# DIAGNijmegen/prostateMR_3D-CAD-csPCa

Hardware: AMD Instinct MI355X
Metric: train-step volumes/sec (whole job), M1 (20,160,160,3) (higher is better)
Workload: dtype bf16; 1 GPU; C3 M1 full hierarchical-probabilistic dense_skip+deep_supervision latents (3,2,1,0) (20,160,160,3); batch_per_gpu=2, global_batch=2, params=67254246, parallelism=dp1, hip_graph=True

## Files before the change

### prostatemr_3d-cad-cspca_amd/csrc/wgrad_tf.hip

```cpp
#include "common.h"
#include "gather.h"
#include <stdlib.h>

typedef __attribute__((ext_vector_type(8))) __bf16 bf16x8_t;
typedef __attribute__((ext_vector_type(4))) float f32x4_t;
typedef short s16x4_t __attribute__((ext_vector_type(4)));
typedef const __attribute__((address_space(1))) void* gptr_t;
typedef __attribute__((address_space(3))) void* lptr_t;

__device__ __attribute__((aligned(64))) unsigned int m1_zero_page_w[16];

__device__ __forceinline__ void glds16w(const void* g, void* lds_wave_base) {
    __builtin_amdgcn_global_load_lds((gptr_t)g, (lptr_t)lds_wave_base, 16, 0, 0);
}
__device__ __forceinline__ s16x4_t tr_read(const unsigned char* p) {
    return __builtin_amdgcn_ds_read_tr16_b64_v4i16((__attribute__((address_space(3))) s16x4_t*)p);
}

#define TF_MAX_NKS 4
#define TF_MAX_AIT 10

struct TfP {
    const bf16_t* A; const bf16_t* B; float* R; float* bsum;
    int CA, CB, AD, AH, AW, BD, BH, BW, N;
    long long RT, RSA; int a_off, b_off;
    int sd, sh, sw, pd, ph, pw;
    int KWs, TH;
    int AHt, AWt;
    int spra, sprb;
    int a_slots, b_slots;
    int a_bytes, b_bytes;
    int tiles_w, tiles_h; long long ntiles;
    int bTiles, nsplit;
    int stages;
    float* Rx; long long rx_stride;
    long long rx_bias;
    int nks;
    int nmem; const bf16_t* Am[M1_MAX_SRC]; long long rx_mem;
};

typedef unsigned u32x2_t __attribute__((ext_vector_type(2)));
__device__ __forceinline__ u32x2_t tr_read_asm(unsigned lds_addr) {
    u32x2_t v;
    asm volatile("ds_read_b64_tr_b16 %0, %1" : "=v"(v) : "v"(lds_addr) : "memory");
    return v;
}
__device__ __forceinline__ void lds_wait2(u32x2_t& a, u32x2_t& b) { asm volatile("s_waitcnt lgkmcnt(0)" : "+v"(a), "+v"(b)); }
__device__ __forceinline__ bf16x8_t frag8(u32x2_t lo, u32x2_t hi) {
    return __builtin_bit_cast(bf16x8_t, __builtin_shufflevector(lo, hi, 0, 1, 2, 3));
}
__device__ __forceinline__ void wait_vm(int n) {
    switch (n) {
#define TF_W(N_) case N_: asm volatile("s_waitcnt vmcnt(" #N_ ")" ::: "memory"); break;
        TF_W(0) TF_W(1) TF_W(2) TF_W(3) TF_W(4) TF_W(5) TF_W(6) TF_W(7) TF_W(8) TF_W(9) TF_W(10) TF_W(11) TF_W(12)
        TF_W(13) TF_W(14) TF_W(15) TF_W(16) TF_W(17) TF_W(18) TF_W(19) TF_W(20) TF_W(21) TF_W(22) TF_W(23) TF_W(24)
        TF_W(25) TF_W(26) TF_W(27) TF_W(28) TF_W(29) TF_W(30) TF_W(31) TF_W(32) TF_W(33) TF_W(34) TF_W(35) TF_W(36)
        TF_W(37) TF_W(38) TF_W(39) TF_W(40) TF_W(41) TF_W(42) TF_W(43) TF_W(44) TF_W(45) TF_W(46) TF_W(47) TF_W(48)
#undef TF_W
        default: asm volatile("s_waitcnt vmcnt(0)" ::: "memory"); break;
    }
}

#define TF_MAX_STAGES 8

template <int KD, int KH, int KW, int KPARTS, int TF_NKS>
__global__ void __launch_bounds__(256) wgrad_tf_kernel(TfP p) {
#if defined(__HIP_DEVICE_COMPILE__)
    constexpr int NT = KD * KH * KW, NG = KD * KH;
    extern __shared__ __attribute__((aligned(16))) unsigned char smem[];
    const int tid = threadIdx.x, lane = tid & 63, wave = __builtin_amdgcn_readfirstlane(tid >> 6);
    constexpr int kparts = KPARTS, ntile = 4 / KPARTS;
    const int ntb = p.CB > 16 ? 2 : 1;
    const int tile_id = wave % ntile, part = wave / ntile;
    const int ta = tile_id / ntb, tb = tile_id % ntb;
    const int a0 = (blockIdx.x / p.bTiles) * 32, b0 = (blockIdx.x % p.bTiles) * 32;
    const int mem = p.nmem > 1 ? (int)blockIdx.z : 0;
    const bf16_t* Abase = p.A;
    if (p.nmem > 1) {
        Abase = p.Am[0];
#pragma unroll
        for (int m = 1; m < M1_MAX_SRC; ++m) if (mem == m) Abase = p.Am[m];
    }
    const int PA = p.spra * 16, PB = p.sprb * 16;
    const int stage_bytes = p.a_bytes + p.b_bytes;
    const unsigned char* zero_pg = reinterpret_cast<const unsigned char*>(m1_zero_page_w);

    constexpr unsigned OOB = 0x80000000u;
    unsigned a_vo[TF_MAX_AIT]; int a_pk[TF_MAX_AIT];
    const int nait = p.a_slots >> 8;
#pragma unroll
    for (int it = 0; it < TF_MAX_AIT; ++it) {
        const int q = it * 256 + tid;
        const int row = q / p.spra, slp = q - row * p.spra;
        const int dd = row / (p.AHt * p.AWt); const int r2 = row - dd * (p.AHt * p.AWt);
        const int hh = r2 / p.AWt, ww = r2 - hh * p.AWt;
        const int sl = p.spra == 4 ? (slp ^ (((ww >> 3) & 1) << 1)) : slp;
        a_pk[it] = dd | (hh << 8) | (ww << 16);
        a_vo[it] = (row < KD * p.AHt * p.AWt) ? (unsigned)((((dd * p.AH + hh) * p.AW + ww) * p.CA + a0 + sl * 8) * 2) : OOB;
    }
    constexpr int NBIT = (TF_NKS * 32 * 4 + 255) / 256;
    const int nbit = (p.b_slots + 255) >> 8;
    unsigned b_vo[NBIT]; int b_th[NBIT];
#pragma unroll
    for (int it = 0; it < NBIT; ++it) {
        const int q = it * 256 + tid;
        const int row = q / p.sprb, slp = q - row * p.sprb;
        const int th = row / p.KWs, tw = row - th * p.KWs;
        const int sl = p.sprb == 4 ? (slp ^ (((tw >> 3) & 1) << 1)) : slp;
        b_th[it] = th;
        b_vo[it] = q < p.b_slots ? (unsigned)(((th * p.BW + tw) * p.CB + b0 + sl * 8) * 2) : OOB;
    }

    int q_kt = blockIdx.y, q_tw, q_th, q_bd, q_n;
    { int r = q_kt; q_tw = r % p.tiles_w; r /= p.tiles_w; q_th = r % p.tiles_h; r /= p.tiles_h; q_bd = r % p.BD; q_n = r / p.BD; }
    int s_tw, s_th, s_bd, s_n;
    { int r = p.nsplit; s_tw = r % p.tiles_w; r /= p.tiles_w; s_th = r % p.tiles_h; r /= p.tiles_h; s_bd = r % p.BD; s_n = r / p.BD; }
    auto issue = [&](int st) {
        const bool live = q_kt < (int)p.ntiles;
        const int twi = q_tw, thi = q_th, bd = q_bd, n = q_n;
        q_kt += p.nsplit;
        q_tw += s_tw; int c = q_tw >= p.tiles_w; q_tw -= c ? p.tiles_w : 0;
        q_th += s_th + c; c = q_th >= p.tiles_h; q_th -= c ? p.tiles_h : 0;
        q_bd += s_bd + c; c = q_bd >= p.BD; q_bd -= c ? p.BD : 0;
        q_n += s_n + c;
        const int ad0 = bd * p.sd - p.pd, ah0 = thi * p.TH * p.sh - p.ph, aw0 = twi * p.KWs * p.sw - p.pw;
        const long long lin0 = (((long long)n * p.AD + ad0) * p.AH + ah0) * p.AW + aw0;
        const int bh0 = thi * p.TH;
        const long long blin0 = (((long long)n * p.BD + bd) * p.BH + bh0) * p.BW + twi * p.KWs;
        unsigned char* As = smem + st * stage_bytes;
        unsigned char* Bs = As + p.a_bytes;
        const __amdgpu_buffer_rsrc_t ra = __builtin_amdgcn_make_buffer_rsrc((void*)(Abase + lin0 * p.CA), 0, live ? 0x7fffffff : 0, 0x00020000);
        const __amdgpu_buffer_rsrc_t rb = __builtin_amdgcn_make_buffer_rsrc((void*)(p.B + blin0 * p.CB), 0, live ? 0x7fffffff : 0, 0x00020000);
        const bool a_inner = ad0 >= 0 && ad0 + KD - 1 < p.AD && ah0 >= 0 && ah0 + p.AHt - 1 < p.AH && aw0 >= 0 && aw0 + p.AWt - 1 < p.AW;
        if (a_inner) {
#pragma unroll
            for (int it = 0; it < TF_MAX_AIT; ++it)
                if (it < nait) __builtin_amdgcn_raw_ptr_buffer_load_lds(ra, (lptr_t)(As + (it * 256 + wave * 64) * 16), 16, a_vo[it], 0, 0, 0);
        } else {
#pragma unroll
            for (int it = 0; it < TF_MAX_AIT; ++it) {
                if (it < nait) {
                    const int pk = a_pk[it];
                    const int dd = pk & 0xff, hh = (pk >> 8) & 0xff, ww = (pk >> 16) & 0xff;
                    const bool ok = (unsigned)(ad0 + dd) < (unsigned)p.AD && (unsigned)(ah0 + hh) < (unsigned)p.AH && (unsigned)(aw0 + ww) < (unsigned)p.AW;
                    __builtin_amdgcn_raw_ptr_buffer_load_lds(ra, (lptr_t)(As + (it * 256 + wave * 64) * 16), 16, ok ? a_vo[it] : OOB, 0, 0, 0);
                }
            }
        }
        const bool b_inner = bh0 + p.TH <= p.BH;
#pragma unroll
        for (int it = 0; it < NBIT; ++it)
            if (it < nbit)
                __builtin_amdgcn_raw_ptr_buffer_load_lds(rb, (lptr_t)(Bs + (it * 256 + wave * 64) * 16), 16,
                                                         (b_inner || bh0 + b_th[it] < p.BH) ? b_vo[it] : OOB, 0, 0, 0);
    };

    const int g = lane >> 4, i = lane & 15;
    const unsigned lds0 = (unsigned)(unsigned long long)(lptr_t)smem;
    unsigned a_ad[TF_NKS][2][KW], b_ad[TF_NKS][2];
#pragma unroll
    for (int ks = 0; ks < TF_NKS; ++ks)
#pragma unroll
        for (int h = 0; h < 2; ++h) {
            const int kk = ks * 32 + 8 * g + 4 * h + (i >> 2);
            const int th = kk / p.KWs, tw = kk - th * p.KWs;
#pragma unroll
            for (int kw = 0; kw < KW; ++kw) {
                const int ww = tw * p.sw + kw;
                const int half = p.spra == 4 ? (ta ^ ((ww >> 3) & 1)) : ta;
                a_ad[ks][h][kw] = lds0 + ((th * p.sh) * p.AWt + ww) * PA + half * 32 + (i & 3) * 8;
            }
            const int halfb = p.sprb == 4 ? (tb ^ ((tw >> 3) & 1)) : tb;
            b_ad[ks][h] = lds0 + p.a_bytes + kk * PB + halfb * 32 + (i & 3) * 8;
        }
    const int grp_pitch = p.AWt * PA;

    f32x4_t acc[NT];
#pragma unroll
    for (int t = 0; t < NT; ++t) acc[t] = (f32x4_t){0.f, 0.f, 0.f, 0.f};
    const bool do_bsum = p.bsum != nullptr && a0 == 0 && ta == 0 && part == 0 && mem == 0;
    f32x4_t accb = (f32x4_t){0.f, 0.f, 0.f, 0.f};
    const bf16x8_t ones = __builtin_bit_cast(bf16x8_t, make_uint4(0x3F803F80u, 0x3F803F80u, 0x3F803F80u, 0x3F803F80u));

    const int S = p.stages;
    const int npiece = nait + nbit;
    const long long kt0 = blockIdx.y, step = p.nsplit;
    for (int s = 0; s < S - 1; ++s) issue(s);
    int st = 0;
    for (long long kt = kt0; kt < p.ntiles; kt += step) {
        wait_vm(npiece * (S - 2));
        __builtin_amdgcn_s_barrier();
        int stn = st + S - 1; if (stn >= S) stn -= S;
        issue(stn);
        const unsigned sb = (unsigned)(st * stage_bytes);
        constexpr int NU = TF_NKS * KD, CH = KH * KW;
        u32x2_t bl[2], bh[2], al[2][CH], ah[2][CH];
        auto rd_unit = [&](int u, int set) {
            const int ks = u / KD, kd = u % KD;
            if (kd == 0) { bl[ks & 1] = tr_read_asm(b_ad[ks][0] + sb); bh[ks & 1] = tr_read_asm(b_ad[ks][1] + sb); }
#pragma unroll
            for (int kh = 0; kh < KH; ++kh) {
                const unsigned ro = sb + (unsigned)((kd * p.AHt + kh) * grp_pitch);
#pragma unroll
                for (int kw = 0; kw < KW; ++kw) {
                    if (((kd * CH + kh * KW + kw) % kparts) == part) {
                        al[set][kh * KW + kw] = tr_read_asm(a_ad[ks][0][kw] + ro);
                        ah[set][kh * KW + kw] = tr_read_asm(a_ad[ks][1][kw] + ro);
                    }
                }
            }
        };
        rd_unit(0, 0);
#pragma unroll
        for (int u = 0; u < NU; ++u) {
            const int ks = u / KD, kd = u % KD, set = u & 1;
            if (kd == 0) lds_wait2(bl[ks & 1], bh[ks & 1]);
#pragma unroll
            for (int c = 0; c < CH; ++c) lds_wait2(al[set][c], ah[set][c]);
            if (u + 1 < NU) rd_unit(u + 1, set ^ 1);
            __builtin_amdgcn_sched_barrier(0);
            const bf16x8_t bfr = frag8(bl[ks & 1], bh[ks & 1]);
            if (do_bsum && kd == 0) accb = __builtin_amdgcn_mfma_f32_16x16x32_bf16(ones, bfr, accb, 0, 0, 0);
#pragma unroll
            for (int c = 0; c < CH; ++c)
                if (((kd * CH + c) % kparts) == part)
                    acc[kd * CH + c] = __builtin_amdgcn_mfma_f32_16x16x32_bf16(frag8(al[set][c], ah[set][c]), bfr, acc[kd * CH + c], 0, 0, 0);
            __builtin_amdgcn_sched_barrier(0);
        }
        if (++st == S) st = 0;
    }
    asm volatile("s_waitcnt vmcnt(0)" ::: "memory");

    float* Rx = p.Rx + (long long)mem * p.rx_mem + (long long)blockIdx.y * p.rx_stride;
    const int b = b0 + tb * 16 + i;
    if (do_bsum && g == 0 && b < p.CB) Rx[p.rx_bias + b] = accb[0];
#pragma unroll
    for (int t = 0; t < NT; ++t)
#pragma unroll
        for (int r = 0; r < 4; ++r) {
            const int a = a0 + ta * 16 + g * 4 + r;
            if ((t % kparts) == part && a < p.CA && b < p.CB) Rx[((long long)t * p.CA + a) * p.CB + b] = acc[t][r];
        }
#endif
}


struct TfFin { float* Rx; long long stride; int ncopies; float* R; int NT, CA, CB; long long RT, RSA; int a_off, b_off;
               float* bsum; long long rx_bias; int nb; int EL; int bias_serial; };
__device__ __forceinline__ void tf_fold_generic(const TfFin& f, unsigned vb, float* red) {
    const long long n = (long long)f.NT * f.CA * f.CB;
    const int e = threadIdx.x % f.EL, y = threadIdx.x / f.EL, YL = 256 / f.EL;
    const long long i = (long long)vb * f.EL + e;
    const long long idx = i;
    float* dst = nullptr;
    if (i < n) {
        const int b = (int)(i % f.CB); const long long q = i / f.CB; const int a = (int)(q % f.CA), t = (int)(q / f.CA);
        dst = f.R + (long long)t * f.RT + (long long)(a + f.a_off) * f.RSA + b + f.b_off;
    } else if (i < n + f.nb) { dst = f.bsum + (i - n) + f.b_off; }
    float s = 0.f;
    if (dst) {
#pragma unroll 8
        for (int c = y; c < f.ncopies; c += YL) s += f.Rx[(long long)c * f.stride + idx];
    }
    red[threadIdx.x] = s;
    __syncthreads();
    if (y == 0 && dst) {
        for (int q = 1; q < YL; ++q) s += red[q * f.EL + e];
        *dst += s;
    }
}
__global__ void __launch_bounds__(256) tf_finish_kernel(TfFin f) {
    __shared__ float red[256];
    tf_fold_generic(f, blockIdx.x, red);
}

__device__ __forceinline__ void tf_fold_vec(const TfFin& f, unsigned vb, unsigned nblk) {
    const long long n = (long long)f.NT * f.CA * f.CB, n4 = n >> 2;
    for (long long q = (long long)vb * 256 + threadIdx.x; q < n4; q += (long long)nblk * 256) {
        const long long i = q << 2;
        float4 s = *reinterpret_cast<const float4*>(f.Rx + i);
        for (int c = 1; c < f.ncopies; ++c) {
            const float4 v = *reinterpret_cast<const float4*>(f.Rx + (long long)c * f.stride + i);
            s.x += v.x; s.y += v.y; s.z += v.z; s.w += v.w;
        }
        const int b = (int)(i % f.CB); const long long r = i / f.CB; const int a = (int)(r % f.CA), t = (int)(r / f.CA);
        float* dst = f.R + (long long)t * f.RT + (long long)(a + f.a_off) * f.RSA + b + f.b_off;
        dst[0] += s.x; dst[1] += s.y; dst[2] += s.z; dst[3] += s.w;
    }
    if (vb == 0)
        for (int j = threadIdx.x; j < f.nb; j += 256) {
            float s = 0.f;
            for (int c = 0; c < f.ncopies; ++c) s += f.Rx[(long long)c * f.stride + n + j];
            f.bsum[j + f.b_off] += s;
        }
}
__global__ void __launch_bounds__(256) tf_finish_vec_kernel(TfFin f) { tf_fold_vec(f, blockIdx.x, gridDim.x); }

__device__ __forceinline__ void tf_fold_wide(const TfFin& f, unsigned vb, float4 (*red)[64]) {
    const long long n = (long long)f.NT * f.CA * f.CB;
    const int lane = threadIdx.x & 63, w = threadIdx.x >> 6;
    const long long i = ((long long)vb * 64 + lane) << 2;
    float4 s = make_float4(0.f, 0.f, 0.f, 0.f);
    if (i < n) {
#pragma unroll 4
        for (int c = w; c < f.ncopies; c += 4) {
            const float4 v = *reinterpret_cast<const float4*>(f.Rx + (long long)c * f.stride + i);
            s.x += v.x; s.y += v.y; s.z += v.z; s.w += v.w;
        }
    }
    red[w][lane] = s;
    __syncthreads();
    if (w == 0 && i < n) {
#pragma unroll
        for (int q = 1; q < 4; ++q) { const float4 v = red[q][lane]; s.x += v.x; s.y += v.y; s.z += v.z; s.w += v.w; }
        const int b = (int)(i % f.CB); const long long r = i / f.CB; const int a = (int)(r % f.CA), t = (int)(r / f.CA);
        float* dst = f.R + (long long)t * f.RT + (long long)(a + f.a_off) * f.RSA + b + f.b_off;
        dst[0] += s.x; dst[1] += s.y; dst[2] += s.z; dst[3] += s.w;
    }
    if (vb == 0 && f.bias_serial) {
        for (int j = threadIdx.x; j < f.nb; j += 256) {
            float sb = 0.f;
            for (int c = 0; c < f.ncopies; ++c) sb += f.Rx[(long long)c * f.stride + n + j];
            f.bsum[j + f.b_off] += sb;
        }
    } else if (vb == 0 && f.nb > 0) {
        __syncthreads();
        float* const rb = reinterpret_cast<float*>(red);
        int nbp = 1; while (nbp < f.nb && nbp < 256) nbp <<= 1;
        const int rows = 256 / nbp, j = threadIdx.x % nbp, r0 = threadIdx.x / nbp;
        for (int j0 = 0; j0 < f.nb; j0 += nbp) {
            float sb = 0.f;
            if (j0 + j < f.nb) {
#pragma unroll 4
                for (int c = r0; c < f.ncopies; c += rows) sb += f.Rx[(long long)c * f.stride + n + j0 + j];
            }
            rb[threadIdx.x] = sb;
            __syncthreads();
            if (r0 == 0 && j0 + j < f.nb) {
                for (int q = 1; q < rows; ++q) sb += rb[q * nbp + j];
                f.bsum[j0 + j + f.b_off] += sb;
            }
            __syncthreads();
        }
    }
}
__global__ void __launch_bounds__(256) tf_finish_wide_kernel(TfFin f) {
    __shared__ float4 red[4][64];
    tf_fold_wide(f, blockIdx.x, red);
}

#define TF_FOLD_MAX 24
struct TfFoldBatch { int n; int pref[TF_FOLD_MAX + 1]; int mode[TF_FOLD_MAX]; TfFin f[TF_FOLD_MAX]; };
static_assert(sizeof(TfFoldBatch) <= 3800, "fold batch must fit the kernel argument segment");
__global__ void __launch_bounds__(256) tf_finish_batch_kernel(TfFoldBatch B) {
    __shared__ float4 red[4][64];
    int j = 0;
    while (j + 1 < B.n && (int)blockIdx.x >= B.pref[j + 1]) ++j;
    const unsigned vb = blockIdx.x - B.pref[j], nblk = B.pref[j + 1] - B.pref[j];
    const TfFin& f = B.f[j];
    if (B.mode[j] == 1) tf_fold_vec(f, vb, nblk);
    else if (B.mode[j] == 2) tf_fold_wide(f, vb, red);
    else tf_fold_generic(f, vb, reinterpret_cast<float*>(red));
}

static inline bool tf_chan_ok(int c) { return c == 8 || c == 16 || (c >= 32 && c % 32 == 0); }

static bool tf_plan(const WgradSpec& g, TfP& p) {
    if (g.dtype != M1_BF16) return false;
    const bool k133 = g.kd == 1 && g.kh == 3 && g.kw == 3, k333 = g.kd == 3 && g.kh == 3 && g.kw == 3;
    if (!k133 && !k333) return false;
    if (!tf_chan_ok(g.CA) || !tf_chan_ok(g.CB)) return false;
    if (g.BW % 8) return false;
    if ((long long)g.N * g.AD * g.AH * g.AW >= (1ll << 31) - (1 << 20) || (long long)g.N * g.BD * g.BH * g.BW >= (1ll << 31) - (1 << 20)) return false;
    p = TfP{};
    p.A = (const bf16_t*)g.A; p.B = (const bf16_t*)g.B; p.R = g.R; p.bsum = g.bsum;
    p.CA = g.CA; p.CB = g.CB; p.AD = g.AD; p.AH = g.AH; p.AW = g.AW; p.BD = g.BD; p.BH = g.BH; p.BW = g.BW; p.N = g.N;
    p.RT = g.RT; p.RSA = g.RSA; p.a_off = g.a_off; p.b_off = g.b_off;
    p.sd = g.sd; p.sh = g.sh; p.sw = g.sw; p.pd = g.pd; p.ph = g.ph; p.pw = g.pw;
    p.KWs = g.BW % 32 == 0 ? 32 : (g.BW % 16 == 0 ? 16 : 8);
    int n4 = M1_CFG("M1_TF_NKS4", 2);
    const int nks = ((n4 && g.CA <= 16 && g.CB <= 16) || (n4 == 2 && g.kd == 1)) ? 4 : 2;
    p.nks = nks;
    p.TH = nks * (32 / p.KWs);
    p.AHt = (p.TH - 1) * g.sh + g.kh; p.AWt = (p.KWs - 1) * g.sw + g.kw;
    p.spra = (g.CA < 32 ? g.CA : 32) / 8; p.sprb = (g.CB < 32 ? g.CB : 32) / 8;
    const int a_rows = g.kd * p.AHt * p.AWt;
    p.a_slots = (a_rows * p.spra + 255) / 256 * 256; p.b_slots = nks * 32 * p.sprb;
    if (p.a_slots > TF_MAX_AIT * 256 || p.AHt > 255 || p.AWt > 255) return false;
    p.a_bytes = p.a_slots * 16; p.b_bytes = (p.b_slots + 255) / 256 * 256 * 16 + 64;
    p.tiles_w = g.BW / p.KWs; p.tiles_h = (g.BH + p.TH - 1) / p.TH;
    p.ntiles = (long long)g.N * g.BD * p.tiles_h * p.tiles_w;
    if (p.ntiles >= (1ll << 30)) return false;
    const int sb = p.a_bytes + p.b_bytes, npiece = p.a_slots / 256 + (p.b_slots + 255) / 256;
    int S = (76 * 1024) / sb;
    if (S < 3) S = 3;
    if (S > TF_MAX_STAGES) S = TF_MAX_STAGES;
    while (S > 3 && npiece * (S - 2) > 48) --S;
    { int fs = M1_CFG("M1_TF_STAGES", 0); if (fs >= 3) S = fs; }
    p.stages = S;
    return npiece * (S - 2) <= 48 && (size_t)S * sb <= 160 * 1024;
}
bool m1_tf_wgrad_supported(const WgradSpec& g) { TfP p; return tf_plan(g, p); }

#include <mutex>
#include <vector>
struct TfPending { TfFin f; int mode; int blocks; };
static std::mutex g_fold_mu;
static std::vector<TfPending> g_fold_pending;
static int g_fold_defer = 0;
static int fold_launch_pending_locked(hipStream_t st) {
    size_t i = 0;
    while (i < g_fold_pending.size()) {
        TfFoldBatch B{}; B.pref[0] = 0;
        while (i < g_fold_pending.size() && B.n < TF_FOLD_MAX) {
            const TfPending& q = g_fold_pending[i++];
            B.f[B.n] = q.f; B.mode[B.n] = q.mode; B.pref[B.n + 1] = B.pref[B.n] + q.blocks; ++B.n;
        }
        hipLaunchKernelGGL(tf_finish_batch_kernel, dim3((unsigned)B.pref[B.n]), dim3(256), 0, st, B);
        int rc = m1_check_launch(); if (rc) { g_fold_pending.clear(); return rc; }
    }
    g_fold_pending.clear();
    return M1_OK;
}
int m1_fold_defer_set(int on) { std::lock_guard<std::mutex> lk(g_fold_mu); const int was = g_fold_defer; g_fold_defer = on ? 1 : 0; return was; }
extern "C" int m1_wgrad_defer(int on) { std::lock_guard<std::mutex> lk(g_fold_mu); g_fold_defer = on ? 1 : 0; return M1_OK; }
int m1_fold_defer_get() { std::lock_guard<std::mutex> lk(g_fold_mu); return g_fold_defer; }
extern "C" int m1_wgrad_fold_drop(void) { { std::lock_guard<std::mutex> lk(g_fold_mu); g_fold_pending.clear(); } m1_colsum_drop_pending(); return M1_OK; }
extern "C" int m1_wgrad_fold_pending(void* stream) {
    if (m1_debug_skip("fold")) return m1_wgrad_fold_drop();
    {
        std::lock_guard<std::mutex> lk(g_fold_mu);
        const int rc = fold_launch_pending_locked((hipStream_t)stream); if (rc) return rc;
    }
    return m1_colsum_launch_pending((hipStream_t)stream);
}

int m1_wg_rx_finish(float* rx, long long stride, int ncopies, const WgradSpec& g, long long nw, hipStream_t st) {
    TfFin f{rx, stride, ncopies, g.R, g.kd * g.kh * g.kw, g.CA, g.CB, g.RT, g.RSA, g.a_off, g.b_off, g.bsum, nw, g.bsum ? g.CB : 0, 32,
            M1_CFG("M1_TF_BIAS_SERIAL", 0)};
    const long long n = (long long)f.NT * f.CA * f.CB + f.nb;
    int mode = 0; long long blocks;
    if (ncopies <= 16 && f.CB % 4 == 0 && n >= (1 << 16)) {
        mode = 1; blocks = (n / 4 + 255) / 256; if (blocks > 4096) blocks = 4096;
    } else if (f.CB % 4 == 0 && n - f.nb >= (1 << 15)) {
        mode = 2; blocks = (n - f.nb + 255) / 256;
    } else {
        while (f.EL > 4 && n / f.EL < 128) f.EL >>= 1;
        blocks = (n + f.EL - 1) / f.EL;
    }
    {
        std::lock_guard<std::mutex> lk(g_fold_mu);
        if (g_fold_defer) {
            bool dup = false;
            for (const TfPending& q : g_fold_pending)
                if (q.f.R == f.R && q.f.a_off == f.a_off && q.f.b_off == f.b_off) { dup = true; break; }
            if (!dup) {
                g_fold_pending.push_back(TfPending{f, mode, (int)blocks});
                return M1_OK;
            }
        }
    }
    if (mode == 1) hipLaunchKernelGGL(tf_finish_vec_kernel, dim3((unsigned)blocks), dim3(256), 0, st, f);
    else if (mode == 2) hipLaunchKernelGGL(tf_finish_wide_kernel, dim3((unsigned)blocks), dim3(256), 0, st, f);
    else hipLaunchKernelGGL(tf_finish_kernel, dim3((unsigned)blocks), dim3(256), 0, st, f);
    return m1_check_launch();
}

#define TF_MAX_COPY_BYTES (96ll << 20)
static int tf_wgrad_launch(const WgradSpec& g, long long nw, int nb, hipStream_t st, int nmem, const void* const* Am, const int* a_offs, long long rx_mem);
int m1_tf_wgrad_multi(const WgradSpec& g, long long nw, int nb, hipStream_t st, int nmem, const void* const* Am, const int* a_offs, long long rx_mem) {
    return tf_wgrad_launch(g, nw, nb, st, nmem, Am, a_offs, rx_mem);
}
int m1_tf_wgrad(const WgradSpec& g, long long nw, int nb, hipStream_t st) { return tf_wgrad_launch(g, nw, nb, st, 1, nullptr, nullptr, 0); }
static int tf_wgrad_launch(const WgradSpec& g, long long nw, int nb, hipStream_t st, int nmem, const void* const* Am, const int* a_offs, long long rx_mem) {
    TfP p;
    if (!tf_plan(g, p)) return M1_ERR_UNSUPPORTED;
    const int TS = 32;
    const int aTiles = (g.CA + TS - 1) / TS; p.bTiles = (g.CB + TS - 1) / TS;
    const int ctiles = aTiles * p.bTiles;
    int tgt_env = M1_CFG("M1_TF_SPLIT", 0);
    const int tgt = tgt_env > 0 ? tgt_env : (p.ntiles >= 24576 ? 512 : 256);
    long long nsplit = (tgt + ctiles - 1) / ctiles;
    const long long nloc = (long long)g.kd * g.kh * g.kw * g.CA * g.CB;
    const long long stride = nloc + g.CB;
    if (nsplit * stride * 4 > TF_MAX_COPY_BYTES) nsplit = TF_MAX_COPY_BYTES / (stride * 4);
    if (!g.rx || g.rx_floats < stride) return M1_ERR_WORKSPACE;
    if (nsplit * stride > g.rx_floats) nsplit = g.rx_floats / stride;
    if (nsplit > p.ntiles) nsplit = p.ntiles;
    if (nsplit < 1) return M1_ERR_UNSUPPORTED;
    p.nsplit = (int)nsplit;
    p.Rx = g.rx; p.rx_stride = stride; p.rx_bias = nloc;
    const size_t smem = (size_t)p.stages * (p.a_bytes + p.b_bytes);
    dim3 grid(ctiles, (unsigned)nsplit, 1);
    p.nmem = 1; p.rx_mem = 0;
    if (nmem > 1) {
        if (nmem > M1_MAX_SRC) return M1_ERR_UNSUPPORTED;
        p.nmem = nmem; p.rx_mem = rx_mem; grid.z = (unsigned)nmem;
        for (int m = 0; m < nmem; ++m) p.Am[m] = (const bf16_t*)Am[m];
    }
    const int kparts = 4 / ((g.CA > 16 ? 2 : 1) * (g.CB > 16 ? 2 : 1));
    void (*kern)(TfP) = nullptr;
#define TF_PICK(KD_, KP_) if ((g.kd == KD_) && kparts == KP_ && p.nks == 2) kern = wgrad_tf_kernel<KD_, 3, 3, KP_, 2>;
    TF_PICK(1, 1) TF_PICK(1, 2) TF_PICK(1, 4) TF_PICK(3, 1) TF_PICK(3, 2) TF_PICK(3, 4)
#undef TF_PICK
    if (p.nks == 4 && kparts == 4) kern = g.kd == 1 ? wgrad_tf_kernel<1, 3, 3, 4, 4> : (g.kd == 3 ? wgrad_tf_kernel<3, 3, 3, 4, 4> : nullptr);
    if (p.nks == 4 && g.kd == 1 && kparts == 1) kern = wgrad_tf_kernel<1, 3, 3, 1, 4>;
    if (p.nks == 4 && g.kd == 1 && kparts == 2) kern = wgrad_tf_kernel<1, 3, 3, 2, 4>;
    if (!kern) return M1_ERR_UNSUPPORTED;
    {
        static const void* done[8]; static int ndone = 0;
        bool seen = false;
        for (int q = 0; q < ndone; ++q) seen |= done[q] == (const void*)kern;
        if (!seen) {
            if (hipFuncSetAttribute((const void*)kern, hipFuncAttributeMaxDynamicSharedMemorySize, 160 * 1024) != hipSuccess) return M1_ERR_LAUNCH;
            if (ndone < 8) done[ndone++] = (const void*)kern;
        }
    }
    m1_note_kernel("wgrad_tf");
    hipLaunchKernelGGL(kern, grid, dim3(256), smem, st, p);
    int rc = m1_check_launch(); if (rc) return rc;
    if (nmem <= 1) return m1_wg_rx_finish(p.Rx, stride, (int)nsplit, g, nloc, st);
    for (int m = 0; m < nmem; ++m) {
        WgradSpec gm = g; gm.a_off = a_offs[m]; if (m) gm.bsum = nullptr;
        rc = m1_wg_rx_finish(p.Rx + (long long)m * rx_mem, stride, (int)nsplit, gm, nloc, st); if (rc) return rc;
    }
    return M1_OK;
}
```

Baseline: 90.35 volumes/s.

## Add kd-ring mode to wgrad kernel reusing depth slices across tiles

Adds a ring-buffer mode for 3x3x3 stride-1 depth weight-gradient kernels. Each block walks a contiguous range of output depth positions and loads only one new input depth slice per step, keeping the previous KD-1 slices resident in LDS instead of reloading all KD slices per tile. This cuts redundant global loads of A by roughly a factor of KD. In exchange it changes the per-block work split from strided to contiguous, adds non-compute warm-up iterations at each depth run, uses a bitmask that assumes fewer than 32 iterations in flight, and falls back to the old path when there are too few tiles per split.

```diff
diff --git a/prostatemr_3d-cad-cspca_amd/csrc/wgrad_tf.hip b/prostatemr_3d-cad-cspca_amd/csrc/wgrad_tf.hip
--- a/prostatemr_3d-cad-cspca_amd/csrc/wgrad_tf.hip
+++ b/prostatemr_3d-cad-cspca_amd/csrc/wgrad_tf.hip
@@ -36,6 +36,7 @@
     float* Rx; long long rx_stride;
     long long rx_bias;
     int nks;
+    int ring, ring_slots;
     int nmem; const bf16_t* Am[M1_MAX_SRC]; long long rx_mem;
 };
 
@@ -63,8 +64,9 @@
 
 #define TF_MAX_STAGES 8
 
-template <int KD, int KH, int KW, int KPARTS, int TF_NKS>
+template <int KD, int KH, int KW, int KPARTS, int TF_NKS, bool RING>
 __global__ void __launch_bounds__(256) wgrad_tf_kernel(TfP p) {
+    static_assert(!RING || KD > 1, "ring mode walks the kd window");
 #if defined(__HIP_DEVICE_COMPILE__)
     constexpr int NT = KD * KH * KW, NG = KD * KH;
     extern __shared__ __attribute__((aligned(16))) unsigned char smem[];
@@ -83,6 +85,7 @@
     }
     const int PA = p.spra * 16, PB = p.sprb * 16;
     const int stage_bytes = p.a_bytes + p.b_bytes;
+    const int ring_a_bytes = p.ring_slots * p.a_bytes;
     const unsigned char* zero_pg = reinterpret_cast<const unsigned char*>(m1_zero_page_w);
 
     constexpr unsigned OOB = 0x80000000u;
@@ -96,7 +99,7 @@
         const int hh = r2 / p.AWt, ww = r2 - hh * p.AWt;
         const int sl = p.spra == 4 ? (slp ^ (((ww >> 3) & 1) << 1)) : slp;
         a_pk[it] = dd | (hh << 8) | (ww << 16);
-        a_vo[it] = (row < KD * p.AHt * p.AWt) ? (unsigned)((((dd * p.AH + hh) * p.AW + ww) * p.CA + a0 + sl * 8) * 2) : OOB;
+        a_vo[it] = (row < (RING ? 1 : KD) * p.AHt * p.AWt) ? (unsigned)((((dd * p.AH + hh) * p.AW + ww) * p.CA + a0 + sl * 8) * 2) : OOB;
     }
     constexpr int NBIT = (TF_NKS * 32 * 4 + 255) / 256;
     const int nbit = (p.b_slots + 255) >> 8;
@@ -155,6 +158,64 @@
                                                          (b_inner || bh0 + b_th[it] < p.BH) ? b_vo[it] : OOB, 0, 0, 0);
     };
 
+    int w_n = 0, w_th = 0, w_tw = 0, w_bd = 0, w_k = 0, niter = 0;
+    if constexpr (RING) {
+        const long long t0 = (long long)blockIdx.y * p.ntiles / p.nsplit, t1 = ((long long)blockIdx.y + 1) * p.ntiles / p.nsplit;
+        if (t1 > t0) niter = (int)(t1 - t0) + (KD - 1) * (int)(1 + (t1 - 1) / p.BD - t0 / p.BD);
+        long long r = t0;
+        w_bd = (int)(r % p.BD); r /= p.BD; w_tw = (int)(r % p.tiles_w); r /= p.tiles_w; w_th = (int)(r % p.tiles_h); w_n = (int)(r / p.tiles_h);
+    }
+    int i_iss = 0, a_slot_iss = 0, b_st_iss = 0;
+    unsigned cmask = 0;
+    auto issue_ring = [&]() {
+        const bool live = i_iss < niter, comp = w_k == KD - 1;
+        const int ad = w_bd * p.sd - p.pd + w_k, ah0 = w_th * p.TH * p.sh - p.ph, aw0 = w_tw * p.KWs * p.sw - p.pw;
+        const bool a_live = live && (unsigned)ad < (unsigned)p.AD;
+        const long long lin0 = (((long long)w_n * p.AD + (a_live ? ad : 0)) * p.AH + ah0) * p.AW + aw0;
+        const int bh0 = w_th * p.TH;
+        const long long blin0 = (((long long)w_n * p.BD + w_bd) * p.BH + bh0) * p.BW + w_tw * p.KWs;
+        unsigned char* As = smem + a_slot_iss * p.a_bytes;
+        unsigned char* Bs = smem + ring_a_bytes + b_st_iss * p.b_bytes;
+        const __amdgpu_buffer_rsrc_t ra = __builtin_amdgcn_make_buffer_rsrc((void*)(Abase + lin0 * p.CA), 0, a_live ? 0x7fffffff : 0, 0x00020000);
+        const __amdgpu_buffer_rsrc_t rb = __builtin_amdgcn_make_buffer_rsrc((void*)(p.B + blin0 * p.CB), 0, (live && comp) ? 0x7fffffff : 0, 0x00020000);
+        const bool a_inner = ah0 >= 0 && ah0 + p.AHt - 1 < p.AH && aw0 >= 0 && aw0 + p.AWt - 1 < p.AW;
+        if (a_inner) {
+#pragma unroll
+            for (int it = 0; it < TF_MAX_AIT; ++it)
+                if (it < nait) __builtin_amdgcn_raw_ptr_buffer_load_lds(ra, (lptr_t)(As + (it * 256 + wave * 64) * 16), 16, a_vo[it], 0, 0, 0);
+        } else {
+#pragma unroll
+            for (int it = 0; it < TF_MAX_AIT; ++it) {
+                if (it < nait) {
+                    const int pk = a_pk[it];
+                    const int hh = (pk >> 8) & 0xff, ww = (pk >> 16) & 0xff;
+                    const bool ok = (unsigned)(ah0 + hh) < (unsigned)p.AH && (unsigned)(aw0 + ww) < (unsigned)p.AW;
+                    __builtin_amdgcn_raw_ptr_buffer_load_lds(ra, (lptr_t)(As + (it * 256 + wave * 64) * 16), 16, ok ? a_vo[it] : OOB, 0, 0, 0);
+                }
+            }
+        }
+        const bool b_inner = bh0 + p.TH <= p.BH;
+#pragma unroll
+        for (int it = 0; it < NBIT; ++it)
+            if (it < nbit)
+                __builtin_amdgcn_raw_ptr_buffer_load_lds(rb, (lptr_t)(Bs + (it * 256 + wave * 64) * 16), 16,
+                                                         (b_inner || bh0 + b_th[it] < p.BH) ? b_vo[it] : OOB, 0, 0, 0);
+        const unsigned bit = 1u << (i_iss & 31);
+        cmask = (live && comp) ? (cmask | bit) : (cmask & ~bit);
+        if (comp) {
+            w_k = KD - 1;
+            if (++w_bd == p.BD) {
+                w_bd = 0; w_k = 0;
+                if (++w_tw == p.tiles_w) { w_tw = 0; if (++w_th == p.tiles_h) { w_th = 0; ++w_n; } }
+            }
+        } else {
+            ++w_k;
+        }
+        ++i_iss;
+        if (++a_slot_iss == p.ring_slots) a_slot_iss = 0;
+        if (++b_st_iss == p.stages) b_st_iss = 0;
+    };
+
     const int g = lane >> 4, i = lane & 15;
     const unsigned lds0 = (unsigned)(unsigned long long)(lptr_t)smem;
     unsigned a_ad[TF_NKS][2][KW], b_ad[TF_NKS][2];
@@ -171,7 +232,7 @@
                 a_ad[ks][h][kw] = lds0 + ((th * p.sh) * p.AWt + ww) * PA + half * 32 + (i & 3) * 8;
             }
             const int halfb = p.sprb == 4 ? (tb ^ ((tw >> 3) & 1)) : tb;
-            b_ad[ks][h] = lds0 + p.a_bytes + kk * PB + halfb * 32 + (i & 3) * 8;
+            b_ad[ks][h] = lds0 + (RING ? ring_a_bytes : p.a_bytes) + kk * PB + halfb * 32 + (i & 3) * 8;
         }
     const int grp_pitch = p.AWt * PA;
 
@@ -184,15 +245,25 @@
 
     const int S = p.stages;
     const int npiece = nait + nbit;
-    const long long kt0 = blockIdx.y, step = p.nsplit;
-    for (int s = 0; s < S - 1; ++s) issue(s);
-    int st = 0;
-    for (long long kt = kt0; kt < p.ntiles; kt += step) {
+    const long long kt0 = RING ? 0 : blockIdx.y, step = RING ? 1 : p.nsplit, kend = RING ? niter : p.ntiles;
+    if constexpr (RING) { for (int s = 0; s < S - 1; ++s) issue_ring(); }
+    else { for (int s = 0; s < S - 1; ++s) issue(s); }
+    int st = 0, a_slot = 0;
+    for (long long kt = kt0; kt < kend; kt += step) {
         wait_vm(npiece * (S - 2));
         __builtin_amdgcn_s_barrier();
         int stn = st + S - 1; if (stn >= S) stn -= S;
-        issue(stn);
-        const unsigned sb = (unsigned)(st * stage_bytes);
+        if constexpr (RING) issue_ring(); else issue(stn);
+        const unsigned sb = (unsigned)(st * (RING ? p.b_bytes : stage_bytes));
+        unsigned a_row0[KD];
+#pragma unroll
+        for (int kd = 0; kd < KD; ++kd) {
+            if constexpr (RING) { int sl = a_slot - (KD - 1) + kd; if (sl < 0) sl += p.ring_slots; a_row0[kd] = (unsigned)(sl * p.a_bytes); }
+            else a_row0[kd] = sb + (unsigned)(kd * p.AHt * grp_pitch);
+        }
+        const bool comp = !RING || ((cmask >> ((int)kt & 31)) & 1);
+        if (RING) { if (++a_slot == p.ring_slots) a_slot = 0; }
+        if (!comp) { if (++st == S) st = 0; continue; }
         constexpr int NU = TF_NKS * KD, CH = KH * KW;
         u32x2_t bl[2], bh[2], al[2][CH], ah[2][CH];
         auto rd_unit = [&](int u, int set) {
@@ -200,7 +271,7 @@
             if (kd == 0) { bl[ks & 1] = tr_read_asm(b_ad[ks][0] + sb); bh[ks & 1] = tr_read_asm(b_ad[ks][1] + sb); }
 #pragma unroll
             for (int kh = 0; kh < KH; ++kh) {
-                const unsigned ro = sb + (unsigned)((kd * p.AHt + kh) * grp_pitch);
+                const unsigned ro = a_row0[kd] + (unsigned)(kh * grp_pitch);
 #pragma unroll
                 for (int kw = 0; kw < KW; ++kw) {
                     if (((kd * CH + kh * KW + kw) % kparts) == part) {
@@ -365,7 +436,7 @@
 
 static inline bool tf_chan_ok(int c) { return c == 8 || c == 16 || (c >= 32 && c % 32 == 0); }
 
-static bool tf_plan(const WgradSpec& g, TfP& p) {
+static bool tf_plan(const WgradSpec& g, TfP& p, bool ring_ok = true) {
     if (g.dtype != M1_BF16) return false;
     const bool k133 = g.kd == 1 && g.kh == 3 && g.kw == 3, k333 = g.kd == 3 && g.kh == 3 && g.kw == 3;
     if (!k133 && !k333) return false;
@@ -398,7 +469,26 @@
     while (S > 3 && npiece * (S - 2) > 48) --S;
     { int fs = M1_CFG("M1_TF_STAGES", 0); if (fs >= 3) S = fs; }
     p.stages = S;
-    return npiece * (S - 2) <= 48 && (size_t)S * sb <= 160 * 1024;
+    if (!(npiece * (S - 2) <= 48 && (size_t)S * sb <= 160 * 1024)) return false;
+    if (ring_ok && g.kd == 3 && g.sd == 1 && M1_CFG("M1_TF_RING", 1)) {
+        const int slice_rows = p.AHt * p.AWt;
+        const int as = (slice_rows * p.spra + 255) / 256 * 256, ab = as * 16, bb = p.b_bytes;
+        const int np = as / 256 + (p.b_slots + 255) / 256;
+        int Sr = (76 * 1024 - (g.kd - 1) * ab) / (ab + bb);
+        if (Sr < 3) Sr = 3;
+        if (Sr > TF_MAX_STAGES) Sr = TF_MAX_STAGES;
+        while (Sr > 3 && np * (Sr - 2) > 48) --Sr;
+        { int fs = M1_CFG("M1_TF_STAGES", 0); if (fs >= 3) Sr = fs; }
+        const size_t lds = (size_t)(Sr + g.kd - 1) * ab + (size_t)Sr * bb;
+        if (np * (Sr - 2) <= 48 && lds <= 160 * 1024) {
+            p.ring = 1; p.ring_slots = Sr + g.kd - 1; p.stages = Sr;
+            p.a_slots = as; p.a_bytes = ab;
+        }
+    }
+    return true;
+}
+static size_t tf_lds_bytes(const TfP& p) {
+    return p.ring ? (size_t)p.ring_slots * p.a_bytes + (size_t)p.stages * p.b_bytes : (size_t)p.stages * (p.a_bytes + p.b_bytes);
 }
 bool m1_tf_wgrad_supported(const WgradSpec& g) { TfP p; return tf_plan(g, p); }
 
@@ -489,8 +579,12 @@
     if (nsplit > p.ntiles) nsplit = p.ntiles;
     if (nsplit < 1) return M1_ERR_UNSUPPORTED;
     p.nsplit = (int)nsplit;
+    if (p.ring && p.ntiles < (long long)M1_CFG("M1_TF_RING_MIN", 24) * nsplit) {
+        if (!tf_plan(g, p, false)) return M1_ERR_UNSUPPORTED;
+        p.bTiles = (g.CB + TS - 1) / TS; p.nsplit = (int)nsplit;
+    }
     p.Rx = g.rx; p.rx_stride = stride; p.rx_bias = nloc;
-    const size_t smem = (size_t)p.stages * (p.a_bytes + p.b_bytes);
+    const size_t smem = tf_lds_bytes(p);
     dim3 grid(ctiles, (unsigned)nsplit, 1);
     p.nmem = 1; p.rx_mem = 0;
     if (nmem > 1) {
@@ -500,20 +594,25 @@
     }
     const int kparts = 4 / ((g.CA > 16 ? 2 : 1) * (g.CB > 16 ? 2 : 1));
     void (*kern)(TfP) = nullptr;
-#define TF_PICK(KD_, KP_) if ((g.kd == KD_) && kparts == KP_ && p.nks == 2) kern = wgrad_tf_kernel<KD_, 3, 3, KP_, 2>;
+#define TF_PICK(KD_, KP_) if ((g.kd == KD_) && kparts == KP_ && p.nks == 2 && !p.ring) kern = wgrad_tf_kernel<KD_, 3, 3, KP_, 2, false>;
     TF_PICK(1, 1) TF_PICK(1, 2) TF_PICK(1, 4) TF_PICK(3, 1) TF_PICK(3, 2) TF_PICK(3, 4)
 #undef TF_PICK
-    if (p.nks == 4 && kparts == 4) kern = g.kd == 1 ? wgrad_tf_kernel<1, 3, 3, 4, 4> : (g.kd == 3 ? wgrad_tf_kernel<3, 3, 3, 4, 4> : nullptr);
-    if (p.nks == 4 && g.kd == 1 && kparts == 1) kern = wgrad_tf_kernel<1, 3, 3, 1, 4>;
-    if (p.nks == 4 && g.kd == 1 && kparts == 2) kern = wgrad_tf_kernel<1, 3, 3, 2, 4>;
+#define TF_PICK_RING(KP_) if (g.kd == 3 && kparts == KP_ && p.nks == 2 && p.ring) kern = wgrad_tf_kernel<3, 3, 3, KP_, 2, true>;
+    TF_PICK_RING(1) TF_PICK_RING(2) TF_PICK_RING(4)
+#undef TF_PICK_RING
+    if (p.nks == 4 && kparts == 4)
+        kern = g.kd == 1 ? wgrad_tf_kernel<1, 3, 3, 4, 4, false>
+                         : (g.kd == 3 ? (p.ring ? wgrad_tf_kernel<3, 3, 3, 4, 4, true> : wgrad_tf_kernel<3, 3, 3, 4, 4, false>) : nullptr);
+    if (p.nks == 4 && g.kd == 1 && kparts == 1) kern = wgrad_tf_kernel<1, 3, 3, 1, 4, false>;
+    if (p.nks == 4 && g.kd == 1 && kparts == 2) kern = wgrad_tf_kernel<1, 3, 3, 2, 4, false>;
     if (!kern) return M1_ERR_UNSUPPORTED;
     {
-        static const void* done[8]; static int ndone = 0;
+        static const void* done[16]; static int ndone = 0;
         bool seen = false;
         for (int q = 0; q < ndone; ++q) seen |= done[q] == (const void*)kern;
         if (!seen) {
             if (hipFuncSetAttribute((const void*)kern, hipFuncAttributeMaxDynamicSharedMemorySize, 160 * 1024) != hipSuccess) return M1_ERR_LAUNCH;
-            if (ndone < 8) done[ndone++] = (const void*)kern;
+            if (ndone < 16) done[ndone++] = (const void*)kern;
         }
     }
     m1_note_kernel("wgrad_tf");
```

Result: no change. 90.09 volumes/s (median of 3 runs) (-0.3%).
